# wyf0912/ContextGS

Hardware: AMD Instinct MI355X
Metric: views/sec fwd+bwd @1920×1080, 1M anchors (higher is better)
Workload: dtype f32

## Files before the change

contextgs_amd/csrc/api.hip:

```cpp
#include <stdarg.h>
#include <string.h>
#include "cgs_internal.h"
#include "raster_forms.h"

static thread_local char g_err[512] = "";

void cgs_set_error(const char *fmt, ...) {
    va_list ap;
    va_start(ap, fmt);
    vsnprintf(g_err, sizeof(g_err), fmt, ap);
    va_end(ap);
}

extern "C" const char *cgs_last_error(void) { return g_err; }
extern "C" int cgs_version(void) { return CGS_VERSION; }
#ifndef CGS_SOURCE_DIGEST
#define CGS_SOURCE_DIGEST "unknown"
#endif
#ifndef CGS_BUILD_FLAGS
#define CGS_BUILD_FLAGS ""
#endif
extern "C" const char *cgs_build_info(void) { return CGS_SOURCE_DIGEST "|" CGS_BUILD_FLAGS; }

int cgs_scan_exclusive_u32_total(const uint32_t *in, uint32_t *out, int64_t n, void *scratch,
// ... 407 lines not shown
    if (mode < 0 || mode > 2) { cgs_set_error("cgs_debug_set_bin_mode: 0 (auto), 1 (radix) or 2 (buckets)"); return CGS_ERR_ARG; }
    g_bin_mode = mode;
    return CGS_OK;
}
static bool use_buckets(const cgs_raster_cfg *cfg, int64_t P, int64_t R) {
    if (g_bin_mode == 1 || !cgs_tile_bin_buckets_ok(cfg) || !cgs_tile_bin_buckets_fits(R)) return false;
    return g_bin_mode == 2 || R >= (int64_t)CGS_BUCKET_MIN_RATIO * P;
}

static int raster_render_impl(const cgs_raster_cfg *cfg, int64_t P, int64_t R, bool spec, void *geom_ws,
                              size_t geom_bytes, void *bin_ws, size_t bin_bytes, void *img_ws,
                              size_t img_bytes, float *out_color, hipStream_t stream) {
    int rc = check_cfg(cfg);
    if (rc) return rc;
    if (!cfg->bg || !out_color || !img_ws) { cgs_set_error("cgs_raster_render: NULL input"); return CGS_ERR_ARG; }
    CgsGeom g;
    CgsBin b;
    CgsImg im;
    memset(&g, 0, sizeof(g));
    memset(&b, 0, sizeof(b));
    const bool bin16 = cgs_tile_bin16_ok(tile_bits(cfg));
    if (spec && (!bin16 || P <= 0 || R <= 0)) {
        cgs_set_error("cgs_raster_render_spec: needs a grid of <= 65536 tiles, P > 0 and a positive capacity");
        return CGS_ERR_ARG;
    }
    if (!cgs_img_carve(&im, img_ws, img_bytes, cfg->image_height, cfg->image_width)) {
        cgs_set_error("image workspace too small");
        return CGS_ERR_WORKSPACE;
    }
    if (P > 0 && (!geom_ws || !cgs_geom_carve(&g, geom_ws, geom_bytes, P))) {
        cgs_set_error("geometry workspace missing or too small");
        return CGS_ERR_WORKSPACE;
    }
    if (R > 0) {
        if (!bin_ws || !cgs_bin_carve(&b, bin_ws, bin_bytes, P, R)) {
            cgs_set_error("binning workspace too small: %zu < %zu", bin_bytes, cgs_raster_bin_bytes(P, R));
            return CGS_ERR_WORKSPACE;
        }
        if (bin16 && use_buckets(cfg, P, R)) {
            if ((rc = cgs_launch_tile_bin_buckets(cfg, P, R, g, b, im, stream, spec ? g.total : nullptr))) return rc;
        } else if (bin16) {
            if ((rc = cgs_launch_tile_bin16(cfg, P, R, tile_bits(cfg), g, b, im, stream, spec ? g.total : nullptr))) return rc;
        } else {
            if ((rc = cgs_launch_emit_pairs(cfg, P, g, b, stream))) return rc;
            CgsProfScope prof(CGS_PROF_TILE_SORT, stream);
            if ((rc = cgs_sort_pairs_u32(b.tile_key_a, b.gid_a, b.tile_key_c, b.gid_sorted, b.tile_key_b, b.gid_b,
                                         R, 0, tile_bits(cfg), b.scratch, b.scratch_bytes, stream)))
                return rc;
        }
    }
    if (!(bin16 && R > 0) && (rc = cgs_launch_ranges(cfg, R, b, im, stream))) return rc;
    if ((rc = cgs_launch_tile_order(cfg, im, stream))) return rc;
    return cgs_launch_blend_fwd(cfg, g, b, im, out_color, stream);
}

extern "C" int cgs_raster_render(const cgs_raster_cfg *cfg, int64_t P, int64_t R, void *geom_ws,
                                 size_t geom_bytes, void *bin_ws, size_t bin_bytes, void *img_ws,
                                 size_t img_bytes, float *out_color, void *stream_) {
    return raster_render_impl(cfg, P, R, false, geom_ws, geom_bytes, bin_ws, bin_bytes, img_ws, img_bytes, out_color,
                              (hipStream_t)stream_);
}

extern "C" int cgs_raster_render_spec(const cgs_raster_cfg *cfg, int64_t P, int64_t R_cap, void *geom_ws,
                                      size_t geom_bytes, void *bin_ws, size_t bin_bytes, void *img_ws,
                                      size_t img_bytes, float *out_color, void *stream_) {
    g_raster_slot.spec_between = true;
    return raster_render_impl(cfg, P, R_cap, true, geom_ws, geom_bytes, bin_ws, bin_bytes, img_ws, img_bytes, out_color,
                              (hipStream_t)stream_);
}

static int raster_backward_blend(const char *fn, const cgs_raster_cfg *cfg, int64_t P, int64_t R, const int32_t *radii,
                                 void *geom_ws, size_t geom_bytes, void *bin_ws, size_t bin_bytes, void *img_ws, size_t img_bytes,
                                 const float *dL_dout, float *dL_dcolors, float *dL_dopacities, void *scratch,
                                 size_t scratch_bytes, CgsGeom &g, float *&d_mean_px, float *&d_conic, hipStream_t stream) {
    int rc;
    if (!dL_dout || !dL_dcolors || !dL_dopacities || !scratch || !radii) {
        cgs_set_error("%s: NULL input", fn);
        return CGS_ERR_ARG;
    }
    if (scratch_bytes < cgs_raster_bwd_scratch_bytes(P)) {
        cgs_set_error("backward scratch too small");
        return CGS_ERR_WORKSPACE;
    }
    CgsBin b;
    CgsImg im;
    memset(&b, 0, sizeof(b));
    if (!geom_ws || !img_ws || !cgs_geom_carve(&g, geom_ws, geom_bytes, P) ||
        !cgs_img_carve(&im, img_ws, img_bytes, cfg->image_height, cfg->image_width)) {
        cgs_set_error("workspace too small");
        return CGS_ERR_WORKSPACE;
    }
    d_mean_px = (float *)scratch;
    d_conic = (float *)((char *)scratch + cgs_align_up(2 * (size_t)P * sizeof(float), 256));
    CGS_CHECK_HIP(hipMemsetAsync(scratch, 0, cgs_raster_bwd_scratch_bytes(P), stream));
    if (R > 0) {
        if (!bin_ws || !cgs_bin_carve(&b, bin_ws, bin_bytes, P, R)) {
            cgs_set_error("binning workspace missing or too small");
            return CGS_ERR_WORKSPACE;
        }
        if ((rc = cgs_launch_blend_bwd(cfg, g, b, im, dL_dout, d_mean_px, d_conic, dL_dopacities, dL_dcolors,
                                       stream)))
            return rc;
    }
    return CGS_OK;
}

extern "C" int cgs_raster_backward(const cgs_raster_cfg *cfg, int64_t P, int64_t R, const float *means3D,
                                   const float *colors, const float *opacities, const float *scales,
                                   const float *rotations, const int32_t *radii, void *geom_ws,
                                   size_t geom_bytes, void *bin_ws, size_t bin_bytes, void *img_ws,
                                   size_t img_bytes, const float *dL_dout, float *dL_dmeans3D,
                                   float *dL_dmeans2D, float *dL_dcolors, float *dL_dopacities,
                                   float *dL_dscales, float *dL_drotations, void *scratch,
                                   size_t scratch_bytes, void *stream_) {
    (void)colors;
    (void)opacities;
    hipStream_t stream = (hipStream_t)stream_;
    int rc = check_cfg(cfg);
    if (rc) return rc;
    if (P == 0) return CGS_OK;
    if (!dL_dmeans3D || !dL_dmeans2D || !dL_dscales || !dL_drotations) {
        cgs_set_error("cgs_raster_backward: NULL input");
        return CGS_ERR_ARG;
    }
    CgsGeom g;
    float *d_mean_px, *d_conic;
    if ((rc = raster_backward_blend("cgs_raster_backward", cfg, P, R, radii, geom_ws, geom_bytes, bin_ws, bin_bytes, img_ws,
// ... 267 lines not shown
```

contextgs_amd/csrc/cgs_internal.h:

```cpp
#pragma once
#include <hip/hip_runtime.h>
#include <stdint.h>
#include <stdio.h>
#include "../../include/cgs.h"

#define CGS_TILE 16
#ifndef CGS_BLEND_BWD_RAW
#define CGS_BLEND_BWD_RAW 0
#endif
#define CGS_WAVE 64

void cgs_set_error(const char *fmt, ...);
uint64_t cgs_new_ticket(int kind);

#define CGS_CHECK_HIP(expr)                                                   \
    do {                                                                      \
        hipError_t e__ = (expr);                                              \
        if (e__ != hipSuccess) {                                              \
            cgs_set_error("%s:%d: %s -> %s", __FILE__, __LINE__, #expr,       \
                          hipGetErrorString(e__));                            \
            return CGS_ERR_HIP;                                               \
        }                                                                     \
    } while (0)

// ... 76 lines not shown
    float *final_T;
    uint32_t *n_contrib;
    uint32_t *tile_last;
    uint32_t *tile_order;
};

size_t cgs_geom_carve(CgsGeom *g, void *ws, size_t bytes, int64_t P);
size_t cgs_bin_carve(CgsBin *b, void *ws, size_t bytes, int64_t P, int64_t R);
size_t cgs_img_carve(CgsImg *im, void *ws, size_t bytes, int32_t H, int32_t W);

int cgs_launch_preprocess(const cgs_raster_cfg *cfg, int64_t P, const float *means3D,
                          const float *colors, const float *opacities, const float *scales,
                          const float *rotations, CgsGeom &g, int32_t *radii, bool filter_only,
                          hipStream_t stream, bool aa = false);
int cgs_launch_emit_pairs(const cgs_raster_cfg *cfg, int64_t P, CgsGeom &g, CgsBin &b,
                          hipStream_t stream);
int cgs_launch_ranges(const cgs_raster_cfg *cfg, int64_t R, CgsBin &b, CgsImg &im,
                      hipStream_t stream);
int cgs_launch_gather_rects(int64_t P, CgsGeom &g, hipStream_t stream);
bool cgs_tile_bin16_ok(int tile_bits);
bool cgs_tile_bin_buckets_ok(const cgs_raster_cfg *cfg);
bool cgs_tile_bin_buckets_fits(int64_t R);
int64_t cgs_bucket_count_slots(int64_t R);
size_t cgs_bucket_tab_words(void);
int cgs_launch_tile_bin_buckets(const cgs_raster_cfg *cfg, int64_t P, int64_t R, CgsGeom &g, CgsBin &b, CgsImg &im,
                                hipStream_t stream, const uint32_t *R_dev);
int cgs_launch_tile_bin16(const cgs_raster_cfg *cfg, int64_t P, int64_t R, int tile_bits, CgsGeom &g, CgsBin &b, CgsImg &im,
                          hipStream_t stream, const uint32_t *R_dev = nullptr);
int cgs_launch_blend_fwd_rows(const cgs_raster_cfg *cfg, CgsGeom &g, CgsBin &b, CgsImg &im, float *out_color,
                              hipStream_t stream);
int cgs_launch_blend_bwd_rows(const cgs_raster_cfg *cfg, CgsGeom &g, CgsBin &b, CgsImg &im, const float *dL_dout,
                              float *dL_dmean2D_px, float *dL_dconic, float *dL_dopacity, float *dL_dcolors,
                              hipStream_t stream);
int cgs_launch_tile_order(const cgs_raster_cfg *cfg, CgsImg &im, hipStream_t stream);
int cgs_launch_blend_fwd(const cgs_raster_cfg *cfg, CgsGeom &g, CgsBin &b, CgsImg &im,
                         float *out_color, hipStream_t stream);
int cgs_launch_blend_bwd(const cgs_raster_cfg *cfg, CgsGeom &g, CgsBin &b, CgsImg &im,
                         const float *dL_dout, float *dL_dmean2D_px, float *dL_dconic,
                         float *dL_dopacity, float *dL_dcolors, hipStream_t stream);
int cgs_launch_preprocess_bwd(const cgs_raster_cfg *cfg, int64_t P, const float4 *rec_raw, const float *means3D,
                              const float *scales, const float *rotations,
                              const int32_t *radii, const float *dL_dmean2D_px,
                              const float *dL_dconic, float *dL_dmeans3D, float *dL_dmeans2D,
                              float *dL_dscales, float *dL_drotations, hipStream_t stream,
                              const float *aa_opacities = nullptr, float *aa_dL_dopacities = nullptr);

struct CgsExpandSrc {
    int64_t n_anchor;
    int K;
    const uint8_t *flags;
    const uint32_t *pos;
    const float *anchor, *gscaling, *offsets, *neural_opacity, *color_in, *cov_in;
    const int64_t *src_row;
};
int cgs_launch_expand_preprocess(const cgs_raster_cfg *cfg, const CgsExpandSrc &x, float *scaling_out, float *xyz_out,
                                 float *rot_out, CgsGeom &g, int32_t *radii, hipStream_t stream);

#ifdef __HIPCC__
__device__ __forceinline__ int64_t cgs_xcd_item(int64_t n_items) {
    const int64_t chunk = (n_items + 7) / 8;
    const int64_t t = (int64_t)(blockIdx.x & 7u) * chunk + (int64_t)(blockIdx.x >> 3);
    return ((int64_t)(blockIdx.x >> 3) < chunk && t < n_items) ? t : -1;
}
#endif
static inline unsigned cgs_xcd_grid(int64_t n_items) { return (unsigned)(8 * ((n_items + 7) / 8)); }
#define CGS_TICKET_SLOTS 8
#define CGS_TICKET_BYTES ((CGS_TICKET_SLOTS + 1) * 128)
// ... 37 lines not shown
```

contextgs_amd/csrc/raster_blend_rows.hip:

```cpp
#include <stdlib.h>
#include <hip/hip_fp16.h>
#include "cgs_internal.h"

#define RB_THREADS 256
#define RB_ALPHA_MIN (1.0f / 255.0f)
#define RB_T_EPS 0.0001f
#define RB_INV_LOG2E 0.6931471805599453f
#define RB_NGRAD 9
#ifndef RB_TILE_ORDER
#define RB_TILE_ORDER 1
#endif
#ifndef RB_XCD_RUN
#define RB_XCD_RUN 0
#endif


namespace {

struct RbEval { float dx, dy, g, alpha; bool hit; };

__device__ __forceinline__ RbEval rb_eval(const float4 r0, const float4 r1, float pxf, float pyf) {
    RbEval e;
    e.dx = r0.x - pxf;
    e.dy = r0.y - pyf;
// ... 328 lines not shown
                const int sub = lane & 15;
                const float red = sub < 4 ? b2[0] : (sub < 8 ? b2[1] : c8);
                if (has && sub < RB_NGRAD && red != 0.f) atomicAdd(&sacc[e][sub], red);
            }
        }
        __syncthreads();
        if (pos < tlast) {
            const float a0 = sacc[tid][0], a1 = sacc[tid][1], a2 = sacc[tid][2], a3 = sacc[tid][3],
                        a4 = sacc[tid][4], a5 = sacc[tid][5], a6 = sacc[tid][6], a7 = sacc[tid][7],
                        a8 = sacc[tid][8];
            if (a0 != 0.f || a1 != 0.f || a2 != 0.f || a3 != 0.f || a4 != 0.f || a5 != 0.f || a6 != 0.f ||
                a7 != 0.f || a8 != 0.f) {
                const uint32_t g = gid_sorted[range.x + pos];
                const float4 q0 = srec[tid * 2], q1 = srec[tid * 2 + 1];
                const float cC = q1.x, op = q1.y;
                atomicAdd(&dL_dmean2D_px[2 * (size_t)g], op * fmaf(2.f * q0.z, a0, q0.w * a1) * RB_INV_LOG2E);
                atomicAdd(&dL_dmean2D_px[2 * (size_t)g + 1], op * fmaf(2.f * cC, a1, q0.w * a0) * RB_INV_LOG2E);
                atomicAdd(&dL_dconic[3 * (size_t)g], -0.5f * op * a2);
                atomicAdd(&dL_dconic[3 * (size_t)g + 1], -op * a3);
                atomicAdd(&dL_dconic[3 * (size_t)g + 2], -0.5f * op * a4);
                atomicAdd(&dL_dopacity[g], a5);
                atomicAdd(&dL_dcolors[3 * (size_t)g], a6);
                atomicAdd(&dL_dcolors[3 * (size_t)g + 1], a7);
                atomicAdd(&dL_dcolors[3 * (size_t)g + 2], a8);
            }
        }
    }
}



#define TO_CLASSES 16
#define TO_THREADS 1024
#ifndef TO_DENSE
#define TO_DENSE 4096u
#endif
#ifndef TO_TOP
#define TO_TOP 13
#endif
__device__ __forceinline__ int to_class(uint32_t len) {
    if (len == 0) return 0;
    const int c = 32 - __clz(len);
    return c < TO_TOP ? c : TO_TOP;
}
__global__ void __launch_bounds__(TO_THREADS) tile_order_kernel(int nt, const uint2 *__restrict__ ranges, uint32_t *__restrict__ order) {
    __shared__ uint32_t cnt[TO_CLASSES][TO_THREADS];
    __shared__ uint32_t wsum[TO_THREADS / 64];
    const int tid = threadIdx.x, lane = tid & 63, wave = tid >> 6;
    const int per = (nt + TO_THREADS - 1) / TO_THREADS;
    const int t0 = tid * per, t1 = min(nt, t0 + per);
#pragma unroll
    for (int c = 0; c < TO_CLASSES; ++c) cnt[c][tid] = 0;
    uint32_t total = 0;
    for (int t = t0; t < t1; ++t) {
        const uint2 r = ranges[t];
        const uint32_t len = r.y > r.x ? r.y - r.x : 0u;
        total += len >> 4;
        cnt[to_class(len)][tid] += 1;
    }
#pragma unroll
    for (int o = 32; o >= 1; o >>= 1) total += __shfl_xor(total, o, 64);
    if (lane == 0) wsum[wave] = total;
    __syncthreads();
    total = 0;
    for (int w = 0; w < TO_THREADS / 64; ++w) total += wsum[w];
    __syncthreads();
    if ((uint64_t)total * 16u > (uint64_t)nt * TO_DENSE) {
        for (int t = t0; t < t1; ++t) order[t] = (uint32_t)t;
        return;
    }
    uint32_t v[TO_CLASSES], mine = 0;
#pragma unroll
    for (int k = 0; k < TO_CLASSES; ++k) {
        const int f = tid * TO_CLASSES + k;
        v[k] = cnt[TO_CLASSES - 1 - f / TO_THREADS][f % TO_THREADS];
        mine += v[k];
    }
    uint32_t inc = mine;
#pragma unroll
    for (int o = 1; o < 64; o <<= 1) {
        const uint32_t up = __shfl_up(inc, o, 64);
        if (lane >= o) inc += up;
    }
    if (lane == 63) wsum[wave] = inc;
    __syncthreads();
    uint32_t run = inc - mine;
    for (int w = 0; w < wave; ++w) run += wsum[w];
    __syncthreads();
#pragma unroll
    for (int k = 0; k < TO_CLASSES; ++k) {
        const int f = tid * TO_CLASSES + k;
        cnt[TO_CLASSES - 1 - f / TO_THREADS][f % TO_THREADS] = run;
        run += v[k];
    }
    __syncthreads();
    for (int t = t0; t < t1; ++t) {
        const uint2 r = ranges[t];
        const int c = to_class(r.y > r.x ? r.y - r.x : 0u);
        order[cnt[c][tid]++] = (uint32_t)t;
    }
}

int cgs_launch_tile_order(const cgs_raster_cfg *cfg, CgsImg &im, hipStream_t stream) {
    const int nt = cgs_tiles_x(cfg) * cgs_tiles_y(cfg);
    hipLaunchKernelGGL(tile_order_kernel, dim3(1), dim3(TO_THREADS), 0, stream, nt, (const uint2 *)im.ranges, im.tile_order);
    CGS_CHECK_LAUNCH(stream, cfg->debug);
    return CGS_OK;
}

int cgs_launch_blend_fwd_rows(const cgs_raster_cfg *cfg, CgsGeom &g, CgsBin &b, CgsImg &im, float *out_color,
                              hipStream_t stream) {
    const int tx = cgs_tiles_x(cfg), ty = cgs_tiles_y(cfg);
    hipLaunchKernelGGL(blend_fwd_rows_kernel, dim3((unsigned)(tx * ty)), dim3(RB_THREADS), 0, stream, cfg->image_width,
                       cfg->image_height, tx, (const uint2 *)im.ranges, (const uint32_t *)b.gid_sorted,
                       (const float4 *)g.rec, cfg->bg, out_color, im.final_T, im.n_contrib, im.tile_last,
                       (const uint32_t *)im.tile_order);
    CGS_CHECK_LAUNCH(stream, cfg->debug);
    return CGS_OK;
}

int cgs_launch_blend_bwd_rows(const cgs_raster_cfg *cfg, CgsGeom &g, CgsBin &b, CgsImg &im, const float *dL_dout,
                              float *dL_dmean2D_px, float *dL_dconic, float *dL_dopacity, float *dL_dcolors,
                              hipStream_t stream) {
    const int tx = cgs_tiles_x(cfg), ty = cgs_tiles_y(cfg);
    const float4 *rec = (const float4 *)g.rec;
    hipLaunchKernelGGL(blend_bwd_rows_kernel, dim3((unsigned)(tx * ty)), dim3(RB_THREADS), 0, stream, cfg->image_width,
                       cfg->image_height, tx, (const uint2 *)im.ranges, (const uint32_t *)b.gid_sorted, rec,
                       cfg->bg, (const float *)im.final_T, (const uint32_t *)im.n_contrib, (const uint32_t *)im.tile_last,
                       dL_dout, dL_dmean2D_px, dL_dconic, dL_dopacity, dL_dcolors, (const uint32_t *)im.tile_order);
    CGS_CHECK_LAUNCH(stream, cfg->debug);
    return CGS_OK;
}
```

contextgs_amd/csrc/tile_bin.hip:

```cpp
#include "cgs_internal.h"
#include "buf_access.h"

#define TB_THREADS 256
#define TB_ITEMS 16
#define TB_TILE (TB_THREADS * TB_ITEMS)
#define TB_WAVES (TB_THREADS / CGS_WAVE)
#define TB_MAXR 256
#ifndef TB_XCD_MAP
#define TB_XCD_MAP 0
#endif

int cgs_scan_exclusive_u32_total(const uint32_t *in, uint32_t *out, int64_t n, void *scratch, size_t scratch_bytes,
                                 uint32_t *grand_total, hipStream_t stream);

namespace {

#ifndef GR_ITEMS
#define GR_ITEMS 2
#endif
#ifndef GR_XCD
#define GR_XCD 1
#endif
__global__ void __launch_bounds__(256)
    gather_rects_kernel(int64_t P, const uint32_t *__restrict__ order, const uint2 *__restrict__ rect,
// ... 92 lines not shown
    const bool some = x1 > x0 && y1 > y0;
    cx0 = x0 / BK_W;
    cy0 = y0 / BK_H;
    cw = some ? (x1 + BK_W - 1) / BK_W - cx0 : 0u;
    ch = some ? (y1 + BK_H - 1) / BK_H - cy0 : 0u;
}

template <bool COARSE>
__device__ __forceinline__ TbPair gen_pair(uint32_t j, uint32_t base, uint32_t i_lo, const uint32_t *sidx,
                                           const uint32_t *__restrict__ offsets, const uint32_t *__restrict__ rect_lo,
                                           const uint32_t *__restrict__ rect_hi, uint32_t tiles_x) {
    TbPair p;
    p.i = i_lo + sidx[j - base];
    p.mask = 0u;
    const uint32_t local = j - offsets[p.i];
    const uint32_t lo = rect_lo[p.i], hi = rect_hi[p.i];
    uint32_t x0 = lo & 0xFFFFu, y0 = lo >> 16, w = (hi & 0xFFFFu) - x0, h = 0;
    if (COARSE) bucket_rect(lo, hi, x0, y0, w, h);
    uint32_t q = (uint32_t)((float)local * __builtin_amdgcn_rcpf((float)w));
    int32_t r = (int32_t)(local - q * w);
    if (r < 0) { --q; r += (int32_t)w; }
    if (r >= (int32_t)w) { ++q; r -= (int32_t)w; }
    p.key = (y0 + q) * tiles_x + x0 + (uint32_t)r;
    if (COARSE) {
        const int32_t tx0 = (int32_t)((x0 + (uint32_t)r) * BK_W), ty0 = (int32_t)((y0 + q) * BK_H);
        const int32_t c0 = max((int32_t)(lo & 0xFFFFu) - tx0, 0), c1 = min((int32_t)(hi & 0xFFFFu) - tx0, BK_W);
        const int32_t r0 = max((int32_t)(lo >> 16) - ty0, 0), r1 = min((int32_t)(hi >> 16) - ty0, BK_H);
        const uint32_t cols = ((1u << c1) - 1u) & ~((1u << c0) - 1u), rows = ((1u << r1) - 1u) & ~((1u << r0) - 1u);
        p.mask = cols * ((rows & 1u) | ((rows & 2u) << 7) | ((rows & 4u) << 14) | ((rows & 8u) << 21));
    }
    return p;
}

template <bool GEN, bool COARSE = false>
__global__ void __launch_bounds__(TB_THREADS)
    tb_hist_kernel(const uint16_t *__restrict__ keys, const uint32_t *__restrict__ offsets,
                   const uint32_t *__restrict__ rect_lo, const uint32_t *__restrict__ rect_hi,
                   const uint32_t *__restrict__ bf, int64_t P, uint32_t R, uint32_t tiles_x,
                   uint32_t *__restrict__ hist , int shift, int nbits, const uint32_t *__restrict__ R_dev,
                   uint32_t ncol, int xcd) {
    const int64_t col_ = xcd ? cgs_xcd_item((int64_t)ncol) : (int64_t)blockIdx.x;
    if (col_ < 0) return;
    const uint32_t col = (uint32_t)col_;
    if (R_dev) R = min(*R_dev, R);
    __shared__ uint32_t h[TB_MAXR];
    __shared__ uint32_t sidx[GEN ? TB_TILE : 1];
    __shared__ uint32_t swave[TB_WAVES];
    const int tid = threadIdx.x;
    const uint32_t mask = (1u << nbits) - 1u;
    h[tid] = 0;
    const uint32_t nblk = (R + (uint32_t)TB_TILE - 1u) / (uint32_t)TB_TILE, per = max(1u, (nblk + ncol - 1u) / ncol);
    const uint32_t b0 = col * per, b1 = min(nblk, b0 + per);
    __syncthreads();
    for (uint32_t blk = b0; blk < b1; ++blk) {
        const uint32_t base = blk * (uint32_t)TB_TILE;
        uint32_t i_lo = 0;
        if (GEN) {
            i_lo = bf[blk];
            build_owner_index(sidx, swave, base, i_lo, bf[blk + 1], P, R, offsets);
        }
#pragma unroll 4
        for (int k = 0; k < TB_ITEMS; ++k) {
            const uint32_t j = base + (uint32_t)(k * TB_THREADS + tid);
            if (j < R) {
                const uint32_t key = GEN ? gen_pair<COARSE>(j, base, i_lo, sidx, offsets, rect_lo, rect_hi, tiles_x).key
                                         : (uint32_t)keys[j];
                atomicAdd(&h[(key >> shift) & mask], 1u);
            }
        }
        __syncthreads();
    }
    if (tid < (1 << nbits)) hist[(int64_t)tid * ncol + col] = h[tid];
}

template <bool GEN, bool FINAL, int NBITS, bool COARSE = false>
__global__ void __launch_bounds__(TB_THREADS)
    tb_scatter_kernel(const uint16_t *__restrict__ keys_in, const uint32_t *__restrict__ vals_in,
                      const uint32_t *__restrict__ offsets, const uint32_t *__restrict__ rect_lo,
                      const uint32_t *__restrict__ rect_hi, const uint32_t *__restrict__ order,
                      const uint32_t *__restrict__ bf, int64_t P, uint32_t R, uint32_t tiles_x,
                      uint16_t *__restrict__ keys_out, uint32_t *__restrict__ vals_out, uint2 *__restrict__ ranges,
                      const uint32_t *__restrict__ hist_scanned, int shift, const uint32_t *__restrict__ R_dev,
                      uint32_t ncol, int xcd, const uint32_t *__restrict__ digit_totals, uint32_t *__restrict__ mask_out = nullptr) {
    const int64_t col_ = xcd ? cgs_xcd_item((int64_t)ncol) : (int64_t)blockIdx.x;
    if (col_ < 0) return;
    const uint32_t col = (uint32_t)col_;
    if (R_dev) R = min(*R_dev, R);
    constexpr int nbits = NBITS;
    const uint32_t nblk = (R + (uint32_t)TB_TILE - 1u) / (uint32_t)TB_TILE, per = max(1u, (nblk + ncol - 1u) / ncol);
    const uint32_t b0 = col * per, b1 = min(nblk, b0 + per);
    if (b0 >= b1) return;
    __shared__ uint32_t wcnt[TB_WAVES][TB_MAXR];
    __shared__ uint32_t lstart[TB_MAXR], gbase[TB_MAXR];
    __shared__ uint32_t wsum[TB_WAVES];
    __shared__ uint32_t stage[TB_TILE + TB_TILE / 2];
    uint32_t *sval = stage;
    uint16_t *skey = (uint16_t *)(stage + TB_TILE);
    const int tid = threadIdx.x, lane = tid & 63, wave = tid >> 6;
    const uint32_t mask = (1u << nbits) - 1u;
    uint32_t gcur = tid < (1 << nbits) ? hist_scanned[(int64_t)tid * ncol + col] : 0u;
    if (digit_totals) {
        const uint32_t gt = tid < (1 << nbits) ? digit_totals[tid] : 0u;
        uint32_t ginc = gt;
#pragma unroll
        for (int o = 1; o < 64; o <<= 1) {
// ... 86 lines not shown
            const uint32_t c = wcnt[w][d];
            wcnt[w][d] = run;
            run += c;
        }
    }
    __syncthreads();
#pragma unroll
    for (int r = 0; r < TB_ITEMS; ++r) {
        const uint32_t j = wbase + (uint32_t)(r * 64 + lane);
        if (j < R) {
            const uint32_t d = (key[r] >> shift) & mask;
            const uint32_t slot = wcnt[wave][d] + rank[r];
            skey[slot] = (uint16_t)key[r];
            sval[slot] = val[r];
            if (COARSE) mask_out[gbase[d] + slot] = tmask[r];
        }
    }
    __syncthreads();
    const int count = (int)min((uint32_t)TB_TILE, R - base);
    for (int j = tid; j < count; j += TB_THREADS) {
        const uint32_t k = skey[j];
        const uint32_t d = (k >> shift) & mask;
        const uint32_t pos = gbase[d] + (uint32_t)j;
        vals_out[pos] = sval[j];
        if (FINAL && !COARSE) {
            if (j + 1 == count || (uint32_t)skey[j + 1] != k) atomicMax(&ranges[k].y, pos + 1u);
        } else if (!FINAL) {
            keys_out[pos] = (uint16_t)k;
        }
    }
    }
}

__global__ void __launch_bounds__(1024) ranges_fix_kernel(int nt, uint2 *__restrict__ ranges) {
    __shared__ uint32_t wmax[16];
    const int tid = threadIdx.x, lane = tid & 63, wave = tid >> 6;
    const int per = (nt + 1023) / 1024;
    const int t0 = tid * per, t1 = min(nt, t0 + per);
    uint32_t run = 0;
    uint32_t y8[8];
#pragma unroll
    for (int k = 0; k < 8; ++k) {
        y8[k] = (per <= 8 && t0 + k < t1) ? ranges[t0 + k].y : 0u;
        run = max(run, y8[k]);
    }
    if (per > 8)
        for (int t = t0; t < t1; ++t) run = max(run, ranges[t].y);
    uint32_t inc = run;
#pragma unroll
    for (int d = 1; d < 64; d <<= 1) {
        const uint32_t o = (uint32_t)__shfl_up((int)inc, d, 64);
        if (lane >= d) inc = max(inc, o);
    }
    if (lane == 63) wmax[wave] = inc;
    __syncthreads();
    uint32_t pre = (uint32_t)__shfl_up((int)inc, 1, 64);
    if (lane == 0) pre = 0;
    for (int w = 0; w < wave; ++w) pre = max(pre, wmax[w]);
    if (per <= 8) {
#pragma unroll
        for (int k = 0; k < 8; ++k)
            if (y8[k]) { ranges[t0 + k].x = pre; pre = y8[k]; }
    } else {
        for (int t = t0; t < t1; ++t) {
            const uint32_t y = ranges[t].y;
            if (y) { ranges[t].x = pre; pre = y; }
        }
    }
}


#define BK_CHUNK 1024
#define BK_THREADS 256
#define BK_WAVES (BK_THREADS / CGS_WAVE)
#define BK_MAXB 256
#define BK_TAB_CR 0
#define BK_TAB_CS 512
#define BK_TAB_NCH 770
#define BK_TAB_TS 1024
#define BK_TAB_WORDS (BK_TAB_TS + BK_MAXB * BK_TILES)

__global__ void __launch_bounds__(256)
    bk_coarse_count_kernel(int64_t P, const uint32_t *__restrict__ rect_lo, const uint32_t *__restrict__ rect_hi,
                           uint32_t *__restrict__ ccnt) {
    const int64_t i = (int64_t)blockIdx.x * 256 + threadIdx.x;
    if (i >= P) return;
    uint32_t cx0, cy0, cw, ch;
    bucket_rect(rect_lo[i], rect_hi[i], cx0, cy0, cw, ch);
    ccnt[i] = cw * ch;
}

__device__ __forceinline__ uint32_t bk_wave_excl_sum(uint32_t v, int lane, uint32_t &total) {
    uint32_t inc = v;
#pragma unroll
    for (int d = 1; d < 64; d <<= 1) {
        const uint32_t o = (uint32_t)__shfl_up((int)inc, d, 64);
        if (lane >= d) inc += o;
    }
    total = (uint32_t)__shfl((int)inc, 63, 64);
    return inc - v;
}

__global__ void __launch_bounds__(256)
    bk_table_kernel(uint32_t *__restrict__ tab, int nbk, uint32_t bx, uint32_t tiles_x, int nt, uint2 *__restrict__ ranges,
// ... 180 lines not shown
    const size_t hist_bytes = cgs_align_up((size_t)TB_MAXR * nb * sizeof(uint32_t), 256);
    if (b.scratch_bytes < hist_bytes + cgs_scan_scratch_bytes((int64_t)TB_MAXR * nb)) {
        cgs_set_error("tile binning: scratch too small");
        return CGS_ERR_WORKSPACE;
    }
    char *scan_scratch = (char *)b.scratch + hist_bytes;
    const size_t scan_bytes = b.scratch_bytes - hist_bytes;
    const uint32_t tiles_x = (uint32_t)cgs_tiles_x(cfg);
    const uint32_t *offsets = g.offsets, *rlo = g.sort_b, *rhi = g.sort_d, *order = g.order;
    int rc;
    uint32_t *totals = (uint32_t *)scan_scratch;
    (void)scan_bytes;
    const unsigned grid = TB_XCD_MAP ? cgs_xcd_grid(nb) : (unsigned)nb;
#define TB_SCATTER_N(GEN, FINAL, N, KIN, VIN, KOUT, VOUT, SHIFT)                                                          \
    hipLaunchKernelGGL((tb_scatter_kernel<GEN, FINAL, N>), dim3(grid), dim3(TB_THREADS), 0, stream, KIN, VIN,             \
                       offsets, rlo, rhi, order, (const uint32_t *)bf, P, (uint32_t)R, tiles_x, KOUT, VOUT, im.ranges,    \
                       (const uint32_t *)hist, SHIFT, R_dev, (uint32_t)nb, TB_XCD_MAP, (const uint32_t *)totals)
#define TB_SCATTER(GEN, FINAL, NB, KIN, VIN, KOUT, VOUT, SHIFT)                                                           \
    do { switch (NB) {                                                                                                    \
        case 1: TB_SCATTER_N(GEN, FINAL, 1, KIN, VIN, KOUT, VOUT, SHIFT); break;                                          \
        case 2: TB_SCATTER_N(GEN, FINAL, 2, KIN, VIN, KOUT, VOUT, SHIFT); break;                                          \
        case 3: TB_SCATTER_N(GEN, FINAL, 3, KIN, VIN, KOUT, VOUT, SHIFT); break;                                          \
        case 4: TB_SCATTER_N(GEN, FINAL, 4, KIN, VIN, KOUT, VOUT, SHIFT); break;                                          \
        case 5: TB_SCATTER_N(GEN, FINAL, 5, KIN, VIN, KOUT, VOUT, SHIFT); break;                                          \
        case 6: TB_SCATTER_N(GEN, FINAL, 6, KIN, VIN, KOUT, VOUT, SHIFT); break;                                          \
        case 7: TB_SCATTER_N(GEN, FINAL, 7, KIN, VIN, KOUT, VOUT, SHIFT); break;                                          \
        default: TB_SCATTER_N(GEN, FINAL, 8, KIN, VIN, KOUT, VOUT, SHIFT); break;                                         \
    } } while (0)
    {
        CgsProfScope prof(CGS_PROF_EMIT_PAIRS, stream);
        const int64_t nthr = nb + 1 > nt ? nb + 1 : nt;
        hipLaunchKernelGGL(block_first_kernel, dim3((unsigned)((nthr + 255) / 256)), dim3(256), 0, stream, nb, P, offsets, bf,
                           nt, im.ranges, R_dev, (uint32_t)R);
        hipLaunchKernelGGL(tb_hist_kernel<true>, dim3(grid), dim3(TB_THREADS), 0, stream,
                           (const uint16_t *)nullptr, offsets, rlo, rhi, (const uint32_t *)bf, P, (uint32_t)R, tiles_x,
                           hist, 0, bits_a, R_dev, (uint32_t)nb, TB_XCD_MAP);
        CGS_CHECK_HIP(hipGetLastError());
        if ((rc = cgs_launch_digit_scan(hist, totals, 1 << bits_a, nb, stream))) return rc;
        if (bits_b)
            TB_SCATTER(true, false, bits_a, (const uint16_t *)nullptr, (const uint32_t *)nullptr, key_a, b.gid_a, 0);
        else
            TB_SCATTER(true, true, bits_a, (const uint16_t *)nullptr, (const uint32_t *)nullptr, (uint16_t *)nullptr,
                       b.gid_sorted, 0);
        CGS_CHECK_LAUNCH(stream, cfg->debug);
    }
    if (bits_b) {
        CgsProfScope prof(CGS_PROF_TILE_SORT, stream);
        hipLaunchKernelGGL(tb_hist_kernel<false>, dim3(grid), dim3(TB_THREADS), 0, stream,
                           (const uint16_t *)key_a, offsets, rlo, rhi, (const uint32_t *)bf, P, (uint32_t)R, tiles_x, hist,
                           bits_a, bits_b, R_dev, (uint32_t)nb, TB_XCD_MAP);
        CGS_CHECK_HIP(hipGetLastError());
        if ((rc = cgs_launch_digit_scan(hist, totals, 1 << bits_b, nb, stream))) return rc;
        TB_SCATTER(false, true, bits_b, (const uint16_t *)key_a, (const uint32_t *)b.gid_a, (uint16_t *)nullptr,
                   b.gid_sorted, bits_a);
        CGS_CHECK_LAUNCH(stream, cfg->debug);
    }
    {
        CgsProfScope prof(CGS_PROF_RANGES, stream);
        hipLaunchKernelGGL(ranges_fix_kernel, dim3(1), dim3(1024), 0, stream, nt, im.ranges);
        CGS_CHECK_LAUNCH(stream, cfg->debug);
    }
    return CGS_OK;
}

static void bk_dims(const cgs_raster_cfg *cfg, uint32_t &bx, uint32_t &by) {
    bx = (uint32_t)(cgs_tiles_x(cfg) + BK_W - 1) / BK_W;
    by = (uint32_t)(cgs_tiles_y(cfg) + BK_H - 1) / BK_H;
}

bool cgs_tile_bin_buckets_ok(const cgs_raster_cfg *cfg) {
    uint32_t bx, by;
    bk_dims(cfg, bx, by);
    return bx * by <= BK_MAXB;
}
bool cgs_tile_bin_buckets_fits(int64_t R) { return R < (1ll << 30) - TB_TILE; }

int64_t cgs_bucket_count_slots(int64_t R) { return (int64_t)BK_TILES * ((R + BK_CHUNK - 1) / BK_CHUNK + BK_MAXB); }
size_t cgs_bucket_tab_words(void) { return BK_TAB_WORDS; }

int cgs_launch_tile_bin_buckets(const cgs_raster_cfg *cfg, int64_t P, int64_t R, CgsGeom &g, CgsBin &b, CgsImg &im,
                                hipStream_t stream, const uint32_t *R_dev) {
    (void)R_dev;
    const int nt = cgs_tiles_x(cfg) * cgs_tiles_y(cfg);
    if (R == 0 || P == 0) {
        CGS_CHECK_HIP(hipMemsetAsync(im.ranges, 0, (size_t)nt * sizeof(uint2), stream));
        return CGS_OK;
    }
    if (!cgs_tile_bin_buckets_fits(R)) { cgs_set_error("tile binning (buckets): pair count out of range"); return CGS_ERR_ARG; }
    uint32_t bx, by;
    bk_dims(cfg, bx, by);
    const int nbk = (int)(bx * by);
    int bits = 1;
    while ((1 << bits) < nbk) ++bits;
    const int64_t nb = (R + TB_TILE - 1) / TB_TILE;
    const int64_t nbc = nb < 2048 ? nb : 2048;
    uint32_t *bf = b.tile_key_b;
    uint32_t *hist = (uint32_t *)b.scratch;
    const size_t hist_bytes = cgs_align_up((size_t)TB_MAXR * nbc * sizeof(uint32_t), 256);
    if (b.scratch_bytes < hist_bytes + cgs_scan_scratch_bytes((int64_t)TB_MAXR * nbc) || !b.bk_tab || !g.sort_c) {
        cgs_set_error("tile binning: scratch too small");
        return CGS_ERR_WORKSPACE;
    }
    char *scan_scratch = (char *)b.scratch + hist_bytes;
    const size_t scan_bytes = b.scratch_bytes - hist_bytes;
    const uint32_t tiles_x = (uint32_t)cgs_tiles_x(cfg), tiles_y = (uint32_t)cgs_tiles_y(cfg);
    const uint32_t *rlo = g.sort_b, *rhi = g.sort_d, *order = g.order;
    uint32_t *coff = g.sort_c, *Rc_dev = g.total + 1;
    uint32_t *tab = b.bk_tab;
    uint2 *cranges = (uint2 *)(tab + BK_TAB_CR);
    uint32_t *cid = b.gid_a, *cmask = b.tile_key_a;
    int rc;
    static const bool tr = getenv("CGS_BK_TRACE") != nullptr;
#define BK_TR(name) do { if (tr) { hipError_t e_ = hipStreamSynchronize(stream); fprintf(stderr, "[bk] %s: %s\n", name, hipGetErrorString(e_)); } } while (0)
    {
        CgsProfScope prof(CGS_PROF_EMIT_PAIRS, stream);
        hipLaunchKernelGGL(bk_coarse_count_kernel, dim3((unsigned)((P + 255) / 256)), dim3(256), 0, stream, P, rlo, rhi, coff);
        CGS_CHECK_HIP(hipGetLastError());
        BK_TR("coarse_count");
        if ((rc = cgs_scan_exclusive_u32_total(coff, coff, P, g.scratch, g.scratch_bytes, Rc_dev, stream))) return rc;
        BK_TR("coarse scan");
        if (tr) { uint32_t h2[2]; hipMemcpy(h2, g.total, 8, hipMemcpyDeviceToHost); fprintf(stderr, "[bk] P %lld, tile pairs %u, bucket pairs %u\n", (long long)P, h2[0], h2[1]); }
        const int64_t nthr = nb + 1 > BK_MAXB ? nb + 1 : BK_MAXB;
        hipLaunchKernelGGL(block_first_kernel, dim3((unsigned)((nthr + 255) / 256)), dim3(256), 0, stream, nb, P,
                           (const uint32_t *)coff, bf, BK_MAXB, cranges, (const uint32_t *)Rc_dev, (uint32_t)R);
        BK_TR("block_first");
        hipLaunchKernelGGL((tb_hist_kernel<true, true>), dim3((unsigned)nbc), dim3(TB_THREADS), 0, stream,
                           (const uint16_t *)nullptr, (const uint32_t *)coff, rlo, rhi, (const uint32_t *)bf, P, (uint32_t)R, bx,
                           hist, 0, bits, (const uint32_t *)Rc_dev, (uint32_t)nbc, 0);
        CGS_CHECK_HIP(hipGetLastError());
        BK_TR("hist");
        if ((rc = cgs_scan_exclusive_u32_total(hist, hist, (int64_t)(1 << bits) * nbc, scan_scratch, scan_bytes, nullptr, stream)))
            return rc;
        BK_TR("hist scan");
#define BK_SCATTER_N(N)                                                                                                   \
    hipLaunchKernelGGL((tb_scatter_kernel<true, true, N, true>), dim3((unsigned)nbc), dim3(TB_THREADS), 0, stream,        \
                       (const uint16_t *)nullptr, (const uint32_t *)nullptr, (const uint32_t *)coff, rlo, rhi, order,     \
                       (const uint32_t *)bf, P, (uint32_t)R, bx, (uint16_t *)nullptr, cid, cranges, (const uint32_t *)hist, 0, \
                       (const uint32_t *)Rc_dev, (uint32_t)nbc, 0, (const uint32_t *)nullptr, cmask)
        switch (bits) {
            case 1: BK_SCATTER_N(1); break;
            case 2: BK_SCATTER_N(2); break;
            case 3: BK_SCATTER_N(3); break;
            case 4: BK_SCATTER_N(4); break;
            case 5: BK_SCATTER_N(5); break;
            case 6: BK_SCATTER_N(6); break;
            case 7: BK_SCATTER_N(7); break;
            default: BK_SCATTER_N(8); break;
        }
        BK_TR("scatter");
        CGS_CHECK_LAUNCH(stream, cfg->debug);
    }
    {
        CgsProfScope prof(CGS_PROF_TILE_SORT, stream);
        hipLaunchKernelGGL(bk_table_kernel, dim3(1), dim3(256), 0, stream, tab, nbk, bx, tiles_x, nt, im.ranges,
                           (const uint32_t *)hist, nbc, 1 << bits, (const uint32_t *)Rc_dev, (uint32_t)R);
        BK_TR("table");
        hipLaunchKernelGGL(bk_count_kernel, dim3(2048), dim3(BK_THREADS), 0, stream, (const uint32_t *)cmask,
                           (const uint32_t *)tab, tiles_x, tiles_y, bx, b.bk_counts);
        CGS_CHECK_HIP(hipGetLastError());
        BK_TR("count");
        if ((rc = cgs_scan_exclusive_u32_total(b.bk_counts, b.bk_scan, cgs_bucket_count_slots(R), b.bk_scan_scratch,
// ... 12 lines not shown
```

Baseline: 160.4.

## Histogram tile pairs per rectangle row and fold range fix into tile-order kernel

```diff
diff --git a/contextgs_amd/csrc/api.hip b/contextgs_amd/csrc/api.hip
--- a/contextgs_amd/csrc/api.hip
+++ b/contextgs_amd/csrc/api.hip
@@ -463,6 +463,7 @@
         cgs_set_error("geometry workspace missing or too small");
         return CGS_ERR_WORKSPACE;
     }
+    bool ends_only = false;
     if (R > 0) {
         if (!bin_ws || !cgs_bin_carve(&b, bin_ws, bin_bytes, P, R)) {
             cgs_set_error("binning workspace too small: %zu < %zu", bin_bytes, cgs_raster_bin_bytes(P, R));
@@ -472,6 +473,7 @@
             if ((rc = cgs_launch_tile_bin_buckets(cfg, P, R, g, b, im, stream, spec ? g.total : nullptr))) return rc;
         } else if (bin16) {
             if ((rc = cgs_launch_tile_bin16(cfg, P, R, tile_bits(cfg), g, b, im, stream, spec ? g.total : nullptr))) return rc;
+            ends_only = true;
         } else {
             if ((rc = cgs_launch_emit_pairs(cfg, P, g, b, stream))) return rc;
             CgsProfScope prof(CGS_PROF_TILE_SORT, stream);
@@ -481,7 +483,7 @@
         }
     }
     if (!(bin16 && R > 0) && (rc = cgs_launch_ranges(cfg, R, b, im, stream))) return rc;
-    if ((rc = cgs_launch_tile_order(cfg, im, stream))) return rc;
+    if ((rc = cgs_launch_tile_order(cfg, im, stream, ends_only))) return rc;
     return cgs_launch_blend_fwd(cfg, g, b, im, out_color, stream);
 }
 
@@ -524,6 +526,7 @@
     d_mean_px = (float *)scratch;
     d_conic = (float *)((char *)scratch + cgs_align_up(2 * (size_t)P * sizeof(float), 256));
     CGS_CHECK_HIP(hipMemsetAsync(scratch, 0, cgs_raster_bwd_scratch_bytes(P), stream));
+    bool ends_only = false;
     if (R > 0) {
         if (!bin_ws || !cgs_bin_carve(&b, bin_ws, bin_bytes, P, R)) {
             cgs_set_error("binning workspace missing or too small");
diff --git a/contextgs_amd/csrc/cgs_internal.h b/contextgs_amd/csrc/cgs_internal.h
--- a/contextgs_amd/csrc/cgs_internal.h
+++ b/contextgs_amd/csrc/cgs_internal.h
@@ -132,7 +132,7 @@
 int cgs_launch_blend_bwd_rows(const cgs_raster_cfg *cfg, CgsGeom &g, CgsBin &b, CgsImg &im, const float *dL_dout,
                               float *dL_dmean2D_px, float *dL_dconic, float *dL_dopacity, float *dL_dcolors,
                               hipStream_t stream);
-int cgs_launch_tile_order(const cgs_raster_cfg *cfg, CgsImg &im, hipStream_t stream);
+int cgs_launch_tile_order(const cgs_raster_cfg *cfg, CgsImg &im, hipStream_t stream, bool fix_starts);
 int cgs_launch_blend_fwd(const cgs_raster_cfg *cfg, CgsGeom &g, CgsBin &b, CgsImg &im,
                          float *out_color, hipStream_t stream);
 int cgs_launch_blend_bwd(const cgs_raster_cfg *cfg, CgsGeom &g, CgsBin &b, CgsImg &im,
diff --git a/contextgs_amd/csrc/raster_blend_rows.hip b/contextgs_amd/csrc/raster_blend_rows.hip
--- a/contextgs_amd/csrc/raster_blend_rows.hip
+++ b/contextgs_amd/csrc/raster_blend_rows.hip
@@ -384,6 +384,7 @@
 
 #define TO_CLASSES 16
 #define TO_THREADS 1024
+#define TO_REG 8
 #ifndef TO_DENSE
 #define TO_DENSE 4096u
 #endif
@@ -395,20 +396,62 @@
     const int c = 32 - __clz(len);
     return c < TO_TOP ? c : TO_TOP;
 }
-__global__ void __launch_bounds__(TO_THREADS) tile_order_kernel(int nt, const uint2 *__restrict__ ranges, uint32_t *__restrict__ order) {
+template <bool FIX_STARTS>
+__global__ void __launch_bounds__(TO_THREADS) tile_order_kernel(int nt, uint2 *ranges, uint32_t *__restrict__ order) {
     __shared__ uint32_t cnt[TO_CLASSES][TO_THREADS];
     __shared__ uint32_t wsum[TO_THREADS / 64];
     const int tid = threadIdx.x, lane = tid & 63, wave = tid >> 6;
     const int per = (nt + TO_THREADS - 1) / TO_THREADS;
     const int t0 = tid * per, t1 = min(nt, t0 + per);
+    const bool in_regs = per <= TO_REG;
+    uint2 r8[TO_REG];
+#pragma unroll
+    for (int k = 0; k < TO_REG; ++k) r8[k] = in_regs && t0 + k < t1 ? ranges[t0 + k] : make_uint2(0u, 0u);
+    if (FIX_STARTS) {
+        uint32_t inc = 0;
+#pragma unroll
+        for (int k = 0; k < TO_REG; ++k) inc = max(inc, r8[k].y);
+        if (!in_regs)
+            for (int t = t0; t < t1; ++t) inc = max(inc, ranges[t].y);
+#pragma unroll
+        for (int d = 1; d < 64; d <<= 1) {
+            const uint32_t o = (uint32_t)__shfl_up((int)inc, d, 64);
+            if (lane >= d) inc = max(inc, o);
+        }
+        if (lane == 63) wsum[wave] = inc;
+        __syncthreads();
+        uint32_t pre = (uint32_t)__shfl_up((int)inc, 1, 64);
+        if (lane == 0) pre = 0;
+        for (int w = 0; w < wave; ++w) pre = max(pre, wsum[w]);
+        __syncthreads();
+        if (in_regs) {
+#pragma unroll
+            for (int k = 0; k < TO_REG; ++k)
+                if (r8[k].y) { r8[k].x = pre; pre = r8[k].y; ranges[t0 + k].x = r8[k].x; }
+        } else {
+            for (int t = t0; t < t1; ++t) {
+                const uint32_t y = ranges[t].y;
+                if (y) { ranges[t].x = pre; pre = y; }
+            }
+        }
+    }
 #pragma unroll
     for (int c = 0; c < TO_CLASSES; ++c) cnt[c][tid] = 0;
     uint32_t total = 0;
-    for (int t = t0; t < t1; ++t) {
-        const uint2 r = ranges[t];
-        const uint32_t len = r.y > r.x ? r.y - r.x : 0u;
-        total += len >> 4;
-        cnt[to_class(len)][tid] += 1;
+    if (in_regs) {
+#pragma unroll
+        for (int k = 0; k < TO_REG; ++k) {
+            const uint32_t len = r8[k].y > r8[k].x ? r8[k].y - r8[k].x : 0u;
+            total += len >> 4;
+            if (t0 + k < t1) cnt[to_class(len)][tid] += 1;
+        }
+    } else {
+        for (int t = t0; t < t1; ++t) {
+            const uint2 r = ranges[t];
+            const uint32_t len = r.y > r.x ? r.y - r.x : 0u;
+            total += len >> 4;
+            cnt[to_class(len)][tid] += 1;
+        }
     }
 #pragma unroll
     for (int o = 32; o >= 1; o >>= 1) total += __shfl_xor(total, o, 64);
@@ -446,6 +489,12 @@
         run += v[k];
     }
     __syncthreads();
+    if (in_regs) {
+#pragma unroll
+        for (int k = 0; k < TO_REG; ++k)
+            if (t0 + k < t1) order[cnt[to_class(r8[k].y > r8[k].x ? r8[k].y - r8[k].x : 0u)][tid]++] = (uint32_t)(t0 + k);
+        return;
+    }
     for (int t = t0; t < t1; ++t) {
         const uint2 r = ranges[t];
         const int c = to_class(r.y > r.x ? r.y - r.x : 0u);
@@ -453,9 +502,14 @@
     }
 }
 
-int cgs_launch_tile_order(const cgs_raster_cfg *cfg, CgsImg &im, hipStream_t stream) {
+int cgs_launch_tile_order(const cgs_raster_cfg *cfg, CgsImg &im, hipStream_t stream, bool fix_starts) {
     const int nt = cgs_tiles_x(cfg) * cgs_tiles_y(cfg);
-    hipLaunchKernelGGL(tile_order_kernel, dim3(1), dim3(TO_THREADS), 0, stream, nt, (const uint2 *)im.ranges, im.tile_order);
+    if (fix_starts) {
+        CgsProfScope prof(CGS_PROF_RANGES, stream);
+        hipLaunchKernelGGL(tile_order_kernel<true>, dim3(1), dim3(TO_THREADS), 0, stream, nt, im.ranges, im.tile_order);
+    } else {
+        hipLaunchKernelGGL(tile_order_kernel<false>, dim3(1), dim3(TO_THREADS), 0, stream, nt, im.ranges, im.tile_order);
+    }
     CGS_CHECK_LAUNCH(stream, cfg->debug);
     return CGS_OK;
 }
diff --git a/contextgs_amd/csrc/tile_bin.hip b/contextgs_amd/csrc/tile_bin.hip
--- a/contextgs_amd/csrc/tile_bin.hip
+++ b/contextgs_amd/csrc/tile_bin.hip
@@ -148,20 +148,14 @@
     return p;
 }
 
-template <bool GEN, bool COARSE = false>
 __global__ void __launch_bounds__(TB_THREADS)
-    tb_hist_kernel(const uint16_t *__restrict__ keys, const uint32_t *__restrict__ offsets,
-                   const uint32_t *__restrict__ rect_lo, const uint32_t *__restrict__ rect_hi,
-                   const uint32_t *__restrict__ bf, int64_t P, uint32_t R, uint32_t tiles_x,
-                   uint32_t *__restrict__ hist , int shift, int nbits, const uint32_t *__restrict__ R_dev,
-                   uint32_t ncol, int xcd) {
+    tb_hist_kernel(const uint16_t *__restrict__ keys, uint32_t R, uint32_t *__restrict__ hist , int shift,
+                   int nbits, const uint32_t *__restrict__ R_dev, uint32_t ncol, int xcd) {
     const int64_t col_ = xcd ? cgs_xcd_item((int64_t)ncol) : (int64_t)blockIdx.x;
     if (col_ < 0) return;
     const uint32_t col = (uint32_t)col_;
     if (R_dev) R = min(*R_dev, R);
     __shared__ uint32_t h[TB_MAXR];
-    __shared__ uint32_t sidx[GEN ? TB_TILE : 1];
-    __shared__ uint32_t swave[TB_WAVES];
     const int tid = threadIdx.x;
     const uint32_t mask = (1u << nbits) - 1u;
     h[tid] = 0;
@@ -170,23 +164,83 @@
     __syncthreads();
     for (uint32_t blk = b0; blk < b1; ++blk) {
         const uint32_t base = blk * (uint32_t)TB_TILE;
-        uint32_t i_lo = 0;
-        if (GEN) {
-            i_lo = bf[blk];
-            build_owner_index(sidx, swave, base, i_lo, bf[blk + 1], P, R, offsets);
-        }
 #pragma unroll 4
         for (int k = 0; k < TB_ITEMS; ++k) {
             const uint32_t j = base + (uint32_t)(k * TB_THREADS + tid);
-            if (j < R) {
-                const uint32_t key = GEN ? gen_pair<COARSE>(j, base, i_lo, sidx, offsets, rect_lo, rect_hi, tiles_x).key
-                                         : (uint32_t)keys[j];
-                atomicAdd(&h[(key >> shift) & mask], 1u);
+            if (j < R) atomicAdd(&h[((uint32_t)keys[j] >> shift) & mask], 1u);
+        }
+    }
+    __syncthreads();
+    if (tid < (1 << nbits)) hist[(int64_t)tid * ncol + col] = h[tid];
+}
+
+template <bool COARSE>
+__global__ void __launch_bounds__(TB_THREADS)
+    tb_hist_rects_kernel(const uint32_t *__restrict__ offsets, const uint32_t *__restrict__ rect_lo,
+                         const uint32_t *__restrict__ rect_hi, const uint32_t *__restrict__ bf, int64_t P, uint32_t R,
+                         uint32_t tiles_x, uint32_t *__restrict__ hist , int nbits,
+                         const uint32_t *__restrict__ R_dev, uint32_t ncol, int xcd) {
+    const int64_t col_ = xcd ? cgs_xcd_item((int64_t)ncol) : (int64_t)blockIdx.x;
+    if (col_ < 0) return;
+    const uint32_t col = (uint32_t)col_;
+    if (R_dev) R = min(*R_dev, R);
+    __shared__ uint32_t h[TB_MAXR], hd[TB_MAXR];
+    __shared__ uint32_t wsum[TB_WAVES];
+    const int tid = threadIdx.x, lane = tid & 63, wave = tid >> 6;
+    const uint32_t N = 1u << nbits, mask = N - 1u;
+    h[tid] = 0;
+    hd[tid] = 0;
+    const uint32_t nblk = (R + (uint32_t)TB_TILE - 1u) / (uint32_t)TB_TILE, per = max(1u, (nblk + ncol - 1u) / ncol);
+    const uint32_t b0 = col * per, b1 = min(nblk, b0 + per);
+    __syncthreads();
+    if (b0 < b1) {
+        const uint32_t base = b0 * (uint32_t)TB_TILE, end = min(R, b1 * (uint32_t)TB_TILE);
+        const uint32_t i_lo = bf[b0], i_hi = bf[b1];
+        for (uint32_t i = i_lo + (uint32_t)tid; i <= i_hi; i += TB_THREADS) {
+            const uint32_t o = offsets[i];
+            const uint32_t on = (int64_t)i + 1 < P ? offsets[i + 1] : R;
+            const uint32_t ja = max(o, base), jb = min(on, end);
+            if (ja >= jb) continue;
+            const uint32_t lo = rect_lo[i], hi = rect_hi[i];
+            uint32_t x0 = lo & 0xFFFFu, y0 = lo >> 16, w = (hi & 0xFFFFu) - x0, hh = 0;
+            if (COARSE) bucket_rect(lo, hi, x0, y0, w, hh);
+            if (w == 0u) continue;
+            uint32_t n = jb - ja;
+            const uint32_t q = ja > o ? (ja - o) / w : 0u, r = (ja - o) - q * w;
+            uint32_t key = (y0 + q) * tiles_x + x0 + r, len = min(w - r, n);
+            while (true) {
+                const uint32_t s = key & mask;
+                if (len == 1u) {
+                    atomicAdd(&h[s], 1u);
+                } else {
+                    const uint32_t turns = len >> nbits, e = s + (len & mask);
+                    if (turns) atomicAdd(&hd[0], turns);
+                    if (e > s) {
+                        atomicAdd(&hd[s], 1u);
+                        if (e > N) atomicAdd(&hd[0], 1u);
+                        if (e != N) atomicAdd(&hd[e & mask], 0xFFFFFFFFu);
+                    }
+                }
+                n -= len;
+                if (n == 0u) break;
+                key += len + tiles_x - w;
+                len = min(w, n);
             }
         }
-        __syncthreads();
-    }
-    if (tid < (1 << nbits)) hist[(int64_t)tid * ncol + col] = h[tid];
+    }
+    __syncthreads();
+    const uint32_t mark = hd[tid];
+    uint32_t inc = mark;
+#pragma unroll
+    for (int o = 1; o < 64; o <<= 1) {
+        const uint32_t up = __shfl_up(inc, o, 64);
+        if (lane >= o) inc += up;
+    }
+    if (lane == 63) wsum[wave] = inc;
+    __syncthreads();
+#pragma unroll
+    for (int w = 0; w < TB_WAVES; ++w) inc += (w < wave) ? wsum[w] : 0u;
+    if (tid < (int)N) hist[(int64_t)tid * ncol + col] = h[tid] + inc;
 }
 
 template <bool GEN, bool FINAL, int NBITS, bool COARSE = false>
@@ -339,44 +393,6 @@
     }
 }
 
-__global__ void __launch_bounds__(1024) ranges_fix_kernel(int nt, uint2 *__restrict__ ranges) {
-    __shared__ uint32_t wmax[16];
-    const int tid = threadIdx.x, lane = tid & 63, wave = tid >> 6;
-    const int per = (nt + 1023) / 1024;
-    const int t0 = tid * per, t1 = min(nt, t0 + per);
-    uint32_t run = 0;
-    uint32_t y8[8];
-#pragma unroll
-    for (int k = 0; k < 8; ++k) {
-        y8[k] = (per <= 8 && t0 + k < t1) ? ranges[t0 + k].y : 0u;
-        run = max(run, y8[k]);
-    }
-    if (per > 8)
-        for (int t = t0; t < t1; ++t) run = max(run, ranges[t].y);
-    uint32_t inc = run;
-#pragma unroll
-    for (int d = 1; d < 64; d <<= 1) {
-        const uint32_t o = (uint32_t)__shfl_up((int)inc, d, 64);
-        if (lane >= d) inc = max(inc, o);
-    }
-    if (lane == 63) wmax[wave] = inc;
-    __syncthreads();
-    uint32_t pre = (uint32_t)__shfl_up((int)inc, 1, 64);
-    if (lane == 0) pre = 0;
-    for (int w = 0; w < wave; ++w) pre = max(pre, wmax[w]);
-    if (per <= 8) {
-#pragma unroll
-        for (int k = 0; k < 8; ++k)
-            if (y8[k]) { ranges[t0 + k].x = pre; pre = y8[k]; }
-    } else {
-        for (int t = t0; t < t1; ++t) {
-            const uint32_t y = ranges[t].y;
-            if (y) { ranges[t].x = pre; pre = y; }
-        }
-    }
-}
-
-
 #define BK_CHUNK 1024
 #define BK_THREADS 256
 #define BK_WAVES (BK_THREADS / CGS_WAVE)
@@ -623,9 +639,8 @@
         const int64_t nthr = nb + 1 > nt ? nb + 1 : nt;
         hipLaunchKernelGGL(block_first_kernel, dim3((unsigned)((nthr + 255) / 256)), dim3(256), 0, stream, nb, P, offsets, bf,
                            nt, im.ranges, R_dev, (uint32_t)R);
-        hipLaunchKernelGGL(tb_hist_kernel<true>, dim3(grid), dim3(TB_THREADS), 0, stream,
-                           (const uint16_t *)nullptr, offsets, rlo, rhi, (const uint32_t *)bf, P, (uint32_t)R, tiles_x,
-                           hist, 0, bits_a, R_dev, (uint32_t)nb, TB_XCD_MAP);
+        hipLaunchKernelGGL(tb_hist_rects_kernel<false>, dim3(grid), dim3(TB_THREADS), 0, stream, offsets, rlo, rhi,
+                           (const uint32_t *)bf, P, (uint32_t)R, tiles_x, hist, bits_a, R_dev, (uint32_t)nb, TB_XCD_MAP);
         CGS_CHECK_HIP(hipGetLastError());
         if ((rc = cgs_launch_digit_scan(hist, totals, 1 << bits_a, nb, stream))) return rc;
         if (bits_b)
@@ -637,18 +652,12 @@
     }
     if (bits_b) {
         CgsProfScope prof(CGS_PROF_TILE_SORT, stream);
-        hipLaunchKernelGGL(tb_hist_kernel<false>, dim3(grid), dim3(TB_THREADS), 0, stream,
-                           (const uint16_t *)key_a, offsets, rlo, rhi, (const uint32_t *)bf, P, (uint32_t)R, tiles_x, hist,
-                           bits_a, bits_b, R_dev, (uint32_t)nb, TB_XCD_MAP);
+        hipLaunchKernelGGL(tb_hist_kernel, dim3(grid), dim3(TB_THREADS), 0, stream, (const uint16_t *)key_a, (uint32_t)R,
+                           hist, bits_a, bits_b, R_dev, (uint32_t)nb, TB_XCD_MAP);
         CGS_CHECK_HIP(hipGetLastError());
         if ((rc = cgs_launch_digit_scan(hist, totals, 1 << bits_b, nb, stream))) return rc;
         TB_SCATTER(false, true, bits_b, (const uint16_t *)key_a, (const uint32_t *)b.gid_a, (uint16_t *)nullptr,
                    b.gid_sorted, bits_a);
-        CGS_CHECK_LAUNCH(stream, cfg->debug);
-    }
-    {
-        CgsProfScope prof(CGS_PROF_RANGES, stream);
-        hipLaunchKernelGGL(ranges_fix_kernel, dim3(1), dim3(1024), 0, stream, nt, im.ranges);
         CGS_CHECK_LAUNCH(stream, cfg->debug);
     }
     return CGS_OK;
@@ -715,9 +724,9 @@
         hipLaunchKernelGGL(block_first_kernel, dim3((unsigned)((nthr + 255) / 256)), dim3(256), 0, stream, nb, P,
                            (const uint32_t *)coff, bf, BK_MAXB, cranges, (const uint32_t *)Rc_dev, (uint32_t)R);
         BK_TR("block_first");
-        hipLaunchKernelGGL((tb_hist_kernel<true, true>), dim3((unsigned)nbc), dim3(TB_THREADS), 0, stream,
-                           (const uint16_t *)nullptr, (const uint32_t *)coff, rlo, rhi, (const uint32_t *)bf, P, (uint32_t)R, bx,
-                           hist, 0, bits, (const uint32_t *)Rc_dev, (uint32_t)nbc, 0);
+        hipLaunchKernelGGL(tb_hist_rects_kernel<true>, dim3((unsigned)nbc), dim3(TB_THREADS), 0, stream,
+                           (const uint32_t *)coff, rlo, rhi, (const uint32_t *)bf, P, (uint32_t)R, bx, hist, bits,
+                           (const uint32_t *)Rc_dev, (uint32_t)nbc, 0);
         CGS_CHECK_HIP(hipGetLastError());
         BK_TR("hist");
         if ((rc = cgs_scan_exclusive_u32_total(hist, hist, (int64_t)(1 << bits) * nbc, scan_scratch, scan_bytes, nullptr, stream)))
```

After: 160.7, median of 5. About the same (+0.2%).
